# savage-hacker14/audio-to-sheet-music

Hardware: AMD Instinct MI355X
Metric: 6s-segments/sec (each separated into 4 stems; encode once, decode 4x) (higher is better)
Workload: dtype bf16; 1 GPU; BASELINE configs[2]: B=64 x 6 s segments x 4 prompts per GPU; global_batch=64, seq_len=264600, prompts=4, parallelism=segment-sharded dp1, launch=hipGraph replay of one athd_forward_prompts per step (1 graph(s) per rank), pipelines=1, decode_items=256

## Files before the change

### audio-to-sheet-music_amd/csrc/forward.cpp

```cpp
#include "forward.h"

namespace athd_fwd {

int forward_impl(athd_ctx* c, const float* wav, int64_t B, int64_t T, const float* text, bool per_item, int P,
                 float* out, void* ws, size_t ws_bytes, void* stream) {
    if (!c) return ATHD_EINVAL;
    if (!c->finalized) return c->fail(ATHD_ESTATE, "athd_forward before athd_finalize");
    if (!wav || !text || !out || B <= 0 || T <= 0 || P <= 0) return c->fail(ATHD_EINVAL, "bad forward arguments");
    if (P > 256) return c->fail(ATHD_EINVAL, "at most 256 prompts per athd_forward_prompts call");
    if (T > (int64_t)1 << 26) return c->fail(ATHD_EINVAL, "segment too long");
    const Dims d = make_dims(c, B, T, P);
    Bufs b;
    Arena sz;
    const size_t need = plan(sz, d, b, c->mode == 1);
    if (!ws || ws_bytes < need) return c->fail(ATHD_EWORKSPACE, "workspace too small: need " + std::to_string(need));
    Arena ar{(char*)ws};
    plan(ar, d, b, c->mode == 1);
    if (hipSetDevice(c->device) != hipSuccess) return c->fail(ATHD_EHIP, "hipSetDevice failed");
    Run r(c, (hipStream_t)stream, b.stats);
    if (hipMemsetAsync(b.stats, 0, (size_t)b.nstats * 2 * sizeof(double), r.s) != hipSuccess)
        return c->fail(ATHD_EHIP, "memset failed");
    struct ProfBind {
        KProf* saved;
        explicit ProfBind(KProf* p) : saved(t_kprof) { t_kprof = p; }
        ~ProfBind() { t_kprof = saved; }
    } prof_bind(c->prof);
    encode(r, d, b, wav);
    if (r.ok()) transformer(r, d, b);
    for (int64_t ch = 0; ch < d.chunks && r.err == 0; ++ch) {
        const int64_t s0 = ch * d.Bc;
        const int64_t bc = std::min(d.Bc, B - s0);
        decode_chunk(r, d, b, s0, bc, text, per_item, out, (ch & 1) && b.FO2 ? b.FO2 : b.FO);
    }
    if (r.ok()) r.sp.final_join();
    if (d.chunks == 1) dump_all(d, b, r.xt2, r.s);
    if (r.err) return c->fail(ATHD_EHIP, "launch failed in " + r.what + " (code " + std::to_string(r.err) + ")");
    hipError_t e = hipGetLastError();
    if (e != hipSuccess) return c->fail(ATHD_EHIP, std::string("HIP error: ") + hipGetErrorString(e));
    return ATHD_OK;
}

}

using namespace athd_fwd;

extern "C" {

size_t athd_workspace_bytes(athd_ctx* c, int64_t B, int64_t T, int P) {
    if (!c || B <= 0 || T <= 0 || P <= 0) return 0;
    Bufs b;
    Arena a;
    return plan(a, make_dims(c, B, T, P), b, c->mode == 1);
}

int athd_forward(athd_ctx* c, const float* wav, int64_t B, int64_t T, const float* text_emb, float* out, void* ws,
                 size_t ws_bytes, void* stream) {
    return forward_impl(c, wav, B, T, text_emb, true, 1, out, ws, ws_bytes, stream);
}

int athd_forward_prompts(athd_ctx* c, const float* wav, int64_t B, int64_t T, const float* text_table, int P,
                         float* out, void* ws, size_t ws_bytes, void* stream) {
    return forward_impl(c, wav, B, T, text_table, false, P, out, ws, ws_bytes, stream);
}

}
```

### audio-to-sheet-music_amd/csrc/forward.h

```cpp
#pragma once
#include <hip/hip_runtime.h>

#include <algorithm>
#include <cstdio>
#include <cstdlib>
#include <string>
#include <vector>

#include "../../include/athd.h"
#include "attn.h"
#include "ctx.h"
#include "gemm.h"
#include "kernels.h"
#include "prof.h"

namespace athd_fwd {

struct Dims {
    int64_t B = 0, T = 0;
    int P = 1, Tspec = 0;
    int F[5] = {2048, 512, 128, 32, 8};
    int64_t L[5] = {0, 0, 0, 0, 0};
    int64_t Nf = 0, Nt = 0, Nmax = 0;
    int64_t Bc = 0, chunks = 0;
};

struct Bufs {
    float* specT;
    double* stats;
    int64_t nstats;
    float *snorm, *tnorm_div, *tnorm_std;
    void *saved[4], *saved_t[4];
    void *sk4, *sk4t;
    void *ybuf, *ybuf_t;
    float *hbuf, *hbuf_t;
    uint16_t *hbuf_b, *hbuf_b_t;
    int ea = 4;
    float *X, *XT;
    void *H[4], *QKV, *O, *F1;
    void *QKVt, *Ot, *F1t;
    float *Gt, *Dt;
    float *pos2d, *pos1d, *x_enc, *xt_enc;
    uint16_t *x_enc_b, *xt_enc_b;
    float *avec, *tc0, *tc2;
    float *Yb, *x_cond, *xt_cond;
    void* Hm;
    float* Ybt;
    void* Hmt;
    float *G, *D, *FO;
    float* FO2 = nullptr;
    float* ola_part;
    LrStep* lrsteps;
    float* gram;
    double* gramq;
    void *S, *Z, *Zs;
    float* skw[2] = {nullptr, nullptr};
};

inline void* eoff(void* p, int64_t n, int ea) { return (char*)p + n * ea; }

struct Switches {
    static bool env(const char* name, bool dflt) {
        const char* e = std::getenv(name);
        return dflt ? !(e && *e == '0') : (e && *e && *e != '0');
    }
    bool serial = env("ATHD_SERIAL", false), sk = env("ATHD_SK", true), rowln = env("ATHD_ROWLN", true),
         fdec1_fused = env("ATHD_FDEC1_FUSED", true), fenc_row = env("ATHD_FENC_ROW", true);
};

struct Status {
    int err = 0;
    std::string what;
    void check(int rc, const char* w) { if (rc != 0 && err == 0) { err = rc; what = w; } }
};

enum Branch { MAIN = 0, TIME = 1 };
struct StreamPlan {
    hipStream_t main, time;
    hipEvent_t ev_f, ev_t;
    bool serial;
    Status* st;

    StreamPlan(athd_ctx* c, hipStream_t caller, bool serial_, Status* st_)
        : main(caller), time(serial_ ? caller : c->s_time), ev_f(c->ev_f), ev_t(c->ev_t), serial(serial_), st(st_) {
        if (!c->s_time || !c->ev_f || !c->ev_t) st->check((int)hipErrorInvalidResourceHandle, "second stream");
    }
    void record(hipEvent_t ev, hipStream_t s) { st->check((int)hipEventRecord(ev, s), "event record"); }
    void wait(hipStream_t s, hipEvent_t ev) { st->check((int)hipStreamWaitEvent(s, ev, 0), "event wait"); }
    void fork() { record(ev_f, main); wait(time, ev_f); }
    void join() { record(ev_t, time); wait(main, ev_t); }
    void cross_join() {
        record(ev_f, main); record(ev_t, time);
        wait(time, ev_f); wait(main, ev_t);
    }
    void main_into_time() { record(ev_f, main); wait(time, ev_f); }
    void chunk_record_time() { if (!serial) record(ev_t, time); }
    void chunk_wait_time() { if (!serial) wait(main, ev_t); }
    void final_join() { if (!serial) join(); }
};

struct Run : Status {
    athd_ctx* c;
    const Switches sw;
    StreamPlan sp;
    hipStream_t s;
    int sk = 0;
    int mode;
    bool actbf;
    double* st_next;
    float* xt2 = nullptr;

    Run(athd_ctx* c_, hipStream_t caller, double* stats_pool)
        : c(c_), sp(c_, caller, sw.serial || c_->prof != nullptr, this), s(caller), mode(c_->mode),
          actbf(c_->mode == 1), st_next(stats_pool) {}
    bool ok() const { return err == 0; }
    double* stats(int64_t pairs) { double* p = st_next; st_next += 2 * pairs; return p; }
    void gemm(const GemmDesc& g, const char* w) {
        KSite site(w);
        check(gemm_launch(g, mode, s), w);
    }
};

struct OnBranch {
    Run& r;
    const hipStream_t saved_s;
    const int saved_sk;
    OnBranch(Run& r_, Branch b) : r(r_), saved_s(r_.s), saved_sk(r_.sk) {
        r.s = b == TIME ? r.sp.time : r.sp.main;
        r.sk = b == TIME && !r.sp.serial ? 1 : 0;
    }
    ~OnBranch() { r.s = saved_s; r.sk = saved_sk; }
};

inline GemmDesc conv_h(const GemmW& w, const void* A, int a_bf16, int64_t nb, int64_t H_in, int64_t W, int C_in,
                       int ntaps, int in_stride, int in_off, int dil, int64_t H_out) {
    GemmDesc g;
    g.A = A; g.a_bf16 = a_bf16; g.nb = (int)nb; g.H_in = (int)H_in; g.W = (int)W; g.C_in = C_in; g.a_ld = C_in;
    g.ntaps = ntaps; g.in_stride = in_stride; g.in_off = in_off; g.dil = dil; g.H_out = (int)H_out;
    g.Wp = w.w; g.N = w.N; g.K = w.K; g.Kp = w.Kp; g.bias = w.bias;
    return g;
}
inline GemmDesc conv1(const GemmW& w, const void* A, int a_bf16, int64_t nb, int64_t H, int64_t W, int C_in) {
    return conv_h(w, A, a_bf16, nb, H, W, C_in, 1, 1, 0, 1, H);
}
inline void out_to(GemmDesc& g, void* C, int c_bf16, int ldo, int64_t H_out_total) {
    g.C = C; g.c_bf16 = c_bf16; g.ldo = ldo; g.H_out_total = (int)H_out_total;
}
inline GemmDesc lin(const GemmW& w, const void* A, int a_bf16, int64_t nb, int64_t ntok, int ldA, void* C, int c_bf16) {
    GemmDesc g = conv1(w, A, a_bf16, nb, ntok, 1, w.K);
    g.a_ld = ldA;
    out_to(g, C, c_bf16, w.N, ntok);
    return g;
}

Dims make_dims(const athd_ctx* c, int64_t B, int64_t T, int P);
size_t plan(Arena& ar, const Dims& d, Bufs& b, bool actbf);
void dump_all(const Dims& d, const Bufs& b, const float* xt2, hipStream_t s);
void encode(Run& r, const Dims& d, const Bufs& b, const float* wav);
void transformer(Run& r, const Dims& d, const Bufs& b);
void decode_chunk(Run& r, const Dims& d, const Bufs& b, int64_t s0, int64_t Bc, const float* text, bool text_per_item,
                  float* out, float* FO);

}
```

### audio-to-sheet-music_amd/csrc/forward_dec.cpp

```cpp
#include "forward.h"

namespace athd_fwd {
namespace {

void conv_t(Run& r, const DecW& w, const void* A, int a_bf16, int nb, int H_in, int W, void* out, int out_bf16,
            double* st, int keep, const char* stage) {
    KStage kst(stage);
    if (w.ct4w && a_bf16 && out_bf16 && convt4_supported(w.cin, w.cout, nb, H_in, W)) {
        ConvT4Desc q;
        q.x = (const uint16_t*)A; q.w = w.ct4w; q.bias = w.ct4b; q.out = (uint16_t*)out; q.stats = st;
        q.nb = nb; q.H = H_in; q.W = W; q.keep = keep < 0 ? 0 : 1;
        r.check(convt4_launch(q, r.s), "convt4");
        return;
    }
    auto residues = [&](const GemmW& gw, int ntaps, int in_off) {
        GemmDesc g = conv_h(gw, A, a_bf16, nb, H_in, W, w.cin, ntaps, 1, in_off, 1, H_in);
        out_to(g, out, out_bf16, w.cout, (keep < 0 ? 4 : 2) * H_in);
        g.o_stride = keep < 0 ? 4 : 2;
        g.stats = st; g.col_split = w.cout;
        return g;
    };
    if (w.quad.w) {
        GemmDesc g = residues(w.quad, 3, -1);
        if (w.cin % 32 == 0) g.k_blk = w.cin;
        if (keep < 0) { g.o_off = 0; g.store_mask = 15; }
        else { g.o_off = -1; g.store_mask = 6; }
        r.gemm(g, "convt.quad");
        return;
    }
    for (int pi = 0; pi < 2; ++pi) {
        GemmDesc g = residues(w.pair[pi], 2, pi == 0 ? -1 : 0);
        if (keep < 0) { g.o_off = 2 * pi; g.store_mask = 3; }
        else if (pi == 0) { g.o_off = 0; g.hi_row_off = 0; g.store_mask = 2; }
        else { g.o_off = 1; g.store_mask = 1; }
        r.gemm(g, pi == 0 ? "convt.pair01" : "convt.pair23");
    }
}

struct Chunk {
    Run& r;
    const Dims& d;
    const Bufs& b;
    athd_ctx* c;
    int64_t s0, Bc;
    int P, NI, ab;
    void text_attn(const float* enc, const uint16_t* enc_b, int64_t ntok, float* cond, void* Hm, float* Yb) const;
    void last_level(DecLastDesc& dl, const float* fold, const void* skip, int64_t H_skip) const {
        dl.NI = NI; dl.P = P;
        dl.fold = fold; dl.skip = skip; dl.skip_bf16 = ab; dl.H_skip = (int)H_skip; dl.C_skip = 4;
    }
    void freq_decoder(float* FO) const;
    float* time_decoder() const;
};

void Chunk::text_attn(const float* enc, const uint16_t* enc_b, int64_t ntok, float* cond, void* Hm, float* Yb) const {
    KStage kst(ntok == d.Nf ? "text_attn.freq" : "text_attn.time");
    GemmDesc g = lin(c->mlp0, enc_b ? (const void*)enc_b : enc, enc_b ? 1 : 0, Bc, ntok, 384, Hm, ab);
    g.bias = nullptr; g.pbias = b.tc0; g.pfold = P; g.act = ACT_GELU;
    r.gemm(g, "text.mlp0");
    GemmDesc g2 = lin(c->mlp2, Hm, ab, NI, ntok, 384, Yb, 0);
    g2.bias = nullptr; g2.pbias = b.tc2; g2.res = enc; g2.res_div = P; g2.res_bs = ntok * 384;
    if (r.actbf) {
        g2.C = cond; g2.c_bf16 = 1; g2.ln_w = c->ta_nw; g2.ln_b = c->ta_nb;
        r.gemm(g2, "text.mlp2.ln");
        return;
    }
    r.gemm(g2, "text.mlp2");
    LnDesc l;
    l.x = Yb; l.nb = NI; l.N = ntok; l.C = 384; l.w = c->ta_nw; l.b = c->ta_nb; l.out = cond; l.out_bf16 = ab;
    layernorm_launch(l, r.s);
}

void Chunk::freq_decoder(float* FO) const {
    const int64_t Ts = d.Tspec;
    const int ea = b.ea;
    void* const sv[4] = {eoff(b.saved[0], s0 * 512 * Ts * 48, ea), eoff(b.saved[1], s0 * 128 * Ts * 96, ea),
                         eoff(b.saved[2], s0 * 32 * Ts * 192, ea), eoff(b.saved[3], s0 * 8 * Ts * 384, ea)};
    double* st = r.stats(NI);
    conv_t(r, c->fdec[0], b.x_cond, ab, NI, 8, (int)Ts, b.G, ab, st, -1, "fdec0");
    KStage kst("fdec0");
    if (r.actbf)
        gn_gelu_bf16in_launch((const uint16_t*)b.G, (uint16_t*)b.S, NI, 32 * Ts * 192, 192, st, c->fdec[0].gnw,
                              c->fdec[0].gnb, r.s);
    else gn_gelu_launch(b.G, NI, 32 * Ts * 192, 192, st, c->fdec[0].gnw, c->fdec[0].gnb, r.s, false);
    KStage kst1("fdec1");
    const DecW& w1 = c->fdec[1];
    GemmDesc gz = conv1(w1.taps, r.actbf ? b.S : (const void*)b.G, ab, NI, 32, Ts, w1.cin);
    out_to(gz, b.Z, ab, w1.taps.N, 32);
    LowRankDesc lr;
    lr.steps = b.lrsteps;
    lr.Z = b.Z; lr.Zs = b.Zs; lr.z_bf16 = ab; lr.Hs = 32; lr.Hk = 8; lr.Hd = (int)Ts; lr.W = (int)Ts;
    lr.Co = w1.cout; lr.P = P; lr.NI = NI; lr.bias = w1.bias; lr.stats = r.stats(NI);
    lr.gn_w = w1.gnw; lr.gn_b = w1.gnb; lr.fast_gelu = ab;
    lr.skip = sv[2]; lr.skip_bf16 = ab; lr.H_skip = 32; lr.C_skip = 192;
    lr.out = b.D; lr.out_bf16 = ab;
    lr.S = gz.A; lr.Wt = w1.taps.w; lr.w_ld = w1.taps.Kp; lr.Ci = w1.cin;
    const bool gram = r.sw.fdec1_fused && b.gram && fdec1_gram_supported(lr);
    if (gram) { lr.z_taps = 4; lr.z4 = b.Z; }
    else r.gemm(gz, "fdec1.z");
    GemmDesc gs = conv1(w1.taps, sv[3], ab, Bc, 8, Ts, w1.cin);
    gs.a_ld = 384;
    out_to(gs, b.Zs, ab, w1.taps.N, 8);
    r.gemm(gs, "fdec1.zs");
    r.check(fdec_lr_steps_launch(b.lrsteps, (int)Ts, 32, 8, 32, r.s), "fdec_lr_steps");
    if (gram) r.check(fdec1_gram_launch(lr, b.gram, b.gramq, r.s), "fdec1_gram");
    else r.check(fdec_lr_stats_launch(lr, r.s), "fdec_lr_stats");
    r.check(fdec_lr_merge_launch(lr, r.s), "fdec_lr_merge");
    const DecW& w = c->fdec[2];
    double* sti = r.stats(NI);
// ... 85 lines not shown
```

### audio-to-sheet-music_amd/csrc/forward_plan.cpp

```cpp
#include "forward.h"

namespace athd_fwd {

Dims make_dims(const athd_ctx* c, int64_t B, int64_t T, int P) {
    Dims d;
    d.B = B; d.T = T; d.P = P;
    d.Tspec = (int)cdiv(T, 1024);
    d.L[0] = T;
    for (int i = 0; i < 4; ++i) d.L[i + 1] = cdiv(d.L[i], 4);
    d.Nf = 8LL * d.Tspec;
    d.Nt = d.L[4];
    d.Nmax = std::max(d.Nf, d.Nt);
    int64_t items_per_chunk = c ? c->decode_items : 64;
    if (const char* e = std::getenv("ATHD_DECODE_ITEMS")) {
        const long v = std::strtol(e, nullptr, 10);
        if (v > 0) items_per_chunk = v;
    }
    d.Bc = std::max<int64_t>(1, std::min<int64_t>(B, items_per_chunk / P));
    d.chunks = cdiv(B, d.Bc);
    return d;
}

size_t plan(Arena& ar, const Dims& d, Bufs& b, bool actbf) {
    const int64_t B = d.B, Ts = d.Tspec;
// ... 32 lines not shown
    b.hbuf_b = ab == 2 ? ar.take<uint16_t>(hmax) : nullptr;
    b.X = ar.take<float>(B * d.Nf * 512);
    b.XT = ar.take<float>(B * d.Nt * 512);
    for (int i = 0; i < 4; ++i) b.H[i] = act(B * d.Nmax * 512);
    b.QKV = act(B * d.Nmax * 1536);
    b.O = act(B * d.Nmax * 512);
    b.F1 = act(B * d.Nmax * 2048);
    b.QKVt = act(B * d.Nmax * 1536);
    b.Ot = act(B * d.Nt * 512);
    b.F1t = act(B * d.Nt * 2048);
    b.pos2d = ar.take<float>(d.Nf * 512);
    b.pos1d = ar.take<float>(d.Nt * 512);
    b.x_enc = ar.take<float>(B * d.Nf * 384);
    b.xt_enc = ar.take<float>(B * d.Nt * 384);
    b.x_enc_b = actbf ? ar.take<uint16_t>(B * d.Nf * 384) : nullptr;
    b.xt_enc_b = actbf ? ar.take<uint16_t>(B * d.Nt * 384) : nullptr;
    const int64_t NI = d.Bc * d.P;
    b.avec = ar.take<float>(NI * 384);
    b.tc0 = ar.take<float>(NI * 384);
    b.tc2 = ar.take<float>(NI * 384);
    b.Hm = act(NI * d.Nf * 384);
    b.Yb = ar.take<float>(NI * d.Nf * 384);
    b.Hmt = act(NI * d.Nt * 384);
    b.Ybt = ar.take<float>(NI * d.Nt * 384);
    b.x_cond = ar.take<float>(NI * d.Nf * 384);
    b.xt_cond = ar.take<float>(NI * d.Nt * 384);
    const int64_t gt = std::max<int64_t>({4 * d.Nt * 192, 4 * d.L[3] * 96, 4 * d.L[2] * 48, d.T * 2});
    const int64_t dmt = std::max<int64_t>({d.L[3] * 192, d.L[2] * 96, d.L[1] * 48});
    b.G = ar.take<float>(NI * std::max<int64_t>({32 * Ts * 192, 2 * Ts * Ts * 96, gt}));
    b.D = ar.take<float>(NI * std::max<int64_t>(Ts * Ts * 192, dmt));
    b.Gt = ar.take<float>(NI * gt);
    b.Dt = ar.take<float>(NI * dmt);
    b.S = act(NI * 32 * Ts * DEC_CH[1]);
    b.Z = act(NI * 32 * Ts * 8 * DEC_CH[2]);
    b.Zs = act(d.Bc * 8 * Ts * 8 * DEC_CH[2]);
    b.FO = ar.take<float>(NI * Ts * Ts * 2);
    if (d.chunks > 1) b.FO2 = ar.take<float>(NI * Ts * Ts * 2);
    b.ola_part = ar.take<float>(istft_ola_part_floats(NI, (int)Ts));
    b.lrsteps = ar.take<LrStep>(Ts + 1);
    b.gram = actbf ? ar.take<float>(fdec1_gram_floats(NI, (int)Ts)) : nullptr;
    b.gramq = actbf ? ar.take<double>(fdec1_gram_q_doubles()) : nullptr;
    for (int i = 0; i < 2; ++i) b.skw[i] = actbf ? ar.take<float>(SK_WS_BYTES / 4) : nullptr;
    return ar.off;
}

static bool dump_dev(const char* dir, const std::string& name, const void* p, size_t n) {
    std::vector<char> h(n);
    if (hipMemcpy(h.data(), p, n, hipMemcpyDeviceToHost) != hipSuccess) return false;
    FILE* f = std::fopen((std::string(dir) + "/" + name).c_str(), "wb");
    if (f) { std::fwrite(h.data(), 1, n, f); std::fclose(f); }
    return true;
}

void dump_all(const Dims& d, const Bufs& b, const float* xt2, hipStream_t s) {
    const char* dir = std::getenv("ATHD_DUMP");
    if (!dir || !*dir) return;
    if (hipStreamSynchronize(s) != hipSuccess) return;
    const int64_t B = d.B, Ts = d.Tspec, NI = std::min(d.B, d.Bc) * d.P;
    struct E { std::string name; const void* p; int64_t n; std::string shape; };
    std::vector<E> es = {
        {"specT", b.specT, B * Ts * 2048 * 4, "B,Ts,2048,4"},
        {"snorm", b.snorm, 2 * B, "B,2"}, {"tnorm_std", b.tnorm_std, 2 * B, "B,2"},
        {"x_enc", b.x_enc, B * d.Nf * 384, "B,Nf,384"}, {"xt_enc", b.xt_enc, B * d.Nt * 384, "B,Nt,384"},
        {"x_cond", b.x_cond, NI * d.Nf * 384, "NI,Nf,384"}, {"xt_cond", b.xt_cond, NI * d.Nt * 384, "NI,Nt,384"},
        {"FO", b.FO, NI * Ts * Ts * 2, "NI,t,row,2"}, {"XT2", xt2, NI * d.T * 2, "NI,T,2"},
    };
    for (int i = 0; i < 4; ++i) {
        const std::string si = std::to_string(i);
        const int64_t nf = B * d.F[i + 1] * Ts * ENC_CH[i], nt = B * d.L[i + 1] * ENC_CH[i];
        if (b.ea == 4) {
            es.push_back({"saved" + si, b.saved[i], nf, "B,F,Ts,C"});
            es.push_back({"saved_t" + si, b.saved_t[i], nt, "B,L,C"});
        } else {
            dump_dev(dir, "saved" + si + ".bf16", b.saved[i], (size_t)nf * 2);
            dump_dev(dir, "saved_t" + si + ".bf16", b.saved_t[i], (size_t)nt * 2);
        }
    }
    struct Rw { const char* name; const void* p; const void* end; };
    const Rw rws[] = {{"G", b.G, b.D}, {"D", b.D, b.Gt}, {"Gt", b.Gt, b.Dt}, {"Dt", b.Dt, b.S}, {"S", b.S, b.Z},
                      {"Z", b.Z, b.Zs}, {"Zs", b.Zs, b.FO}, {"stats", b.stats, b.specT}};
    for (const auto& e : rws)
        if (e.p && e.end && e.end > e.p)
            dump_dev(dir, std::string(e.name) + ".raw", e.p, (size_t)((const char*)e.end - (const char*)e.p));
    FILE* fi = std::fopen((std::string(dir) + "/index.txt").c_str(), "w");
    for (const auto& e : es)
        if (dump_dev(dir, e.name + ".f32", e.p, (size_t)e.n * 4) && fi)
            std::fprintf(fi, "%s %lld %s\n", e.name.c_str(), (long long)e.n, e.shape.c_str());
    if (fi) std::fclose(fi);
}

}
```

### audio-to-sheet-music_amd/csrc/forward_xf.cpp

```cpp
#include "forward.h"

namespace athd_fwd {
namespace {

struct Pending { const double* st = nullptr; const float* w = nullptr; const float* b = nullptr; };

struct BranchX {
    float* X;
    int64_t N;
    void *QKV, *O, *F1;
    Pending pend;
    Pending resgn;
};

struct Xf {
    Run& r;
    const Dims& d;
    const Bufs& b;
    const int ab;

    void ln(BranchX& x, const float* w, const float* bb, bool pending, void* out, const float* w2 = nullptr,
            const float* b2 = nullptr, void* out2 = nullptr) {
        LnDesc l;
        l.x = x.X; l.nb = (int)d.B; l.N = x.N; l.C = 512; l.w = w; l.b = bb; l.out = out; l.out_bf16 = ab;
// ... 6 lines not shown
        l.w2 = w2; l.b2 = b2; l.out2 = out2;
        layernorm_launch(l, r.s);
    }
    void block(const TLayerW& L, BranchX& x, void* Hq, void* Hkv, int64_t Nk) {
        const int64_t B = d.B, N = x.N;
        AttnDesc a;
        a.nb = (int)B; a.Nq = (int)N; a.Nk = (int)Nk; a.heads = 8;
        a.scale = r.actbf ? ATTN_SCALE_PRESCALED : 0.125f;
        if (!L.cross) {
            r.gemm(lin(L.qkv, Hq, ab, B, N, 512, x.QKV, ab), "qkv");
            a.Q = x.QKV; a.q_bf16 = ab; a.q_bs = N * 1536; a.q_ld = 1536; a.q_off = 0;
            a.K = x.QKV; a.k_bf16 = ab; a.k_bs = N * 1536; a.k_ld = 1536; a.k_off = 512;
            a.V = x.QKV; a.v_bf16 = ab; a.v_bs = N * 1536; a.v_ld = 1536; a.v_off = 1024;
        } else {
            char* Qb = (char*)x.QKV;
            char* KVb = Qb + (size_t)B * d.Nmax * 512 * (ab ? 2 : 4);
            r.gemm(lin(L.q, Hq, ab, B, N, 512, Qb, ab), "q");
            r.gemm(lin(L.kv, Hkv, ab, B, Nk, 512, KVb, ab), "kv");
            a.Q = Qb; a.q_bf16 = ab; a.q_bs = N * 512; a.q_ld = 512; a.q_off = 0;
            a.K = KVb; a.k_bf16 = ab; a.k_bs = Nk * 1024; a.k_ld = 1024; a.k_off = 0;
            a.V = KVb; a.v_bf16 = ab; a.v_bs = Nk * 1024; a.v_ld = 1024; a.v_off = 512;
        }
        a.O = x.O; a.o_bf16 = ab; a.o_bs = N * 512; a.o_ld = 512;
        r.check(attn_launch(a, r.mode, r.s), "attention");
        GemmDesc go = lin(L.out, x.O, ab, B, N, 512, x.X, 0);
        go.res = x.X; go.res_scale = L.g1;
        if (x.resgn.st) {
            go.res_gn_stats = x.resgn.st; go.res_gn_count = N * 512; go.res_gn_w = x.resgn.w; go.res_gn_b = x.resgn.b;
            x.resgn = Pending();
        }
        const float *n2w = L.cross ? L.n3w : L.n2w, *n2b = L.cross ? L.n3b : L.n2b;
        go.ln_w = n2w; go.ln_b = n2b; go.ln_out = Hq;
        if (r.actbf && r.sw.rowln && rowln_supported(go)) {
            r.gemm(go, "out_proj.ln");
        } else {
            go.ln_w = go.ln_b = nullptr; go.ln_out = nullptr;
            r.gemm(go, "out_proj");
            ln(x, n2w, n2b, false, Hq);
        }
        GemmDesc g1 = lin(L.l1, Hq, ab, B, N, 512, x.F1, ab);
        g1.act = ACT_GELU;
        r.gemm(g1, "linear1");
        double* st = r.stats(B);
        GemmDesc g2 = lin(L.l2, x.F1, ab, B, N, 2048, x.X, 0);
        g2.res = x.X; g2.res_scale = L.g2; g2.stats = st;
        g2.sk_ws = r.sw.sk ? b.skw[r.sk] : nullptr;
        r.gemm(g2, "linear2");
        x.pend.st = st; x.pend.w = L.now; x.pend.b = L.nob;
    }
    void down(const GemmW& w, BranchX& x, float* enc, uint16_t* enc_b, const char* site) {
        GemmDesc g = lin(w, x.X, 0, d.B, x.N, 512, enc, 0);
        if (r.actbf) { g.a_gn_stats = x.pend.st; g.a_gn_count = x.N * 512; g.a_gn_w = x.pend.w; g.a_gn_b = x.pend.b; }
        r.gemm(g, site);
        if (enc_b) to_bf16_launch(enc, enc_b, d.B * x.N * 384, r.s);
    }
};

}

void transformer(Run& r, const Dims& d, const Bufs& b) {
    athd_ctx* c = r.c;
    KStage xstage("transformer");
    KSection sec_x("transformer");
    const int64_t B = d.B;
    Xf xf{r, d, b, r.actbf ? 1 : 0};
    BranchX f{b.X, d.Nf, b.QKV, b.O, b.F1}, t{b.XT, d.Nt, b.QKVt, b.Ot, b.F1t};
    r.gemm(lin(c->up, b.saved[3], xf.ab, B, d.Nf, 384, b.X, 0), "upsampler");
    r.gemm(lin(c->up_t, b.saved_t[3], xf.ab, B, d.Nt, 384, b.XT, 0), "upsampler_t");
    pos2d_launch(b.pos2d, 8, d.Tspec, 512, r.s);
    pos1d_launch(b.pos1d, (int)d.Nt, 512, r.s);
    LnDesc l;
    l.x = b.X; l.nb = (int)B; l.N = d.Nf; l.C = 512; l.w = c->nin_w; l.b = c->nin_b; l.pos = b.pos2d; l.out = b.X;
    layernorm_launch(l, r.s);
    LnDesc lt;
    lt.x = b.XT; lt.nb = (int)B; lt.N = d.Nt; lt.C = 512; lt.w = c->nint_w; lt.b = c->nint_b; lt.pos = b.pos1d; lt.out = b.XT;
    layernorm_launch(lt, r.s);
    if (!r.ok()) return;
    r.sp.fork();
    for (int idx = 0; idx < 5; ++idx) {
        const TLayerW& Lf = c->L[idx];
        const TLayerW& Lt = c->Lt[idx];
        if (!Lf.cross) {
            xf.ln(f, Lf.n1w, Lf.n1b, true, b.H[0]);
            xf.block(Lf, f, b.H[0], nullptr, d.Nf);
            OnBranch on(r, TIME);
            xf.ln(t, Lt.n1w, Lt.n1b, true, b.H[2]);
            xf.block(Lt, t, b.H[2], nullptr, d.Nt);
        } else {
            r.sp.cross_join();
            xf.ln(f, Lf.n1w, Lf.n1b, true, b.H[0], Lt.n2w, Lt.n2b, b.H[1]);
            {
                OnBranch on(r, TIME);
                xf.ln(t, Lt.n1w, Lt.n1b, true, b.H[2], Lf.n2w, Lf.n2b, b.H[3]);
            }
            r.sp.cross_join();
            xf.block(Lf, f, b.H[0], b.H[3], d.Nt);
            OnBranch on(r, TIME);
            xf.block(Lt, t, b.H[2], b.H[1], d.Nf);
        }
    }
    if (!r.actbf) gn_apply_launch(b.X, (int)B, d.Nf, 512, f.pend.st, f.pend.w, f.pend.b, r.s);
    {
        OnBranch on(r, TIME);
        if (!r.actbf) gn_apply_launch(b.XT, (int)B, d.Nt, 512, t.pend.st, t.pend.w, t.pend.b, r.s);
        xf.down(c->down_t, t, b.xt_enc, b.xt_enc_b, "downsampler_t");
    }
    xf.down(c->down, f, b.x_enc, b.x_enc_b, "downsampler");
// ... 5 lines not shown
```

### audio-to-sheet-music_amd/csrc/kernels.h

```cpp
#pragma once
#include <hip/hip_runtime.h>
#include <stdint.h>

#include "gemm.h"

namespace athd {

struct PadPlan {
    int64_t L;
    int64_t left;
    int64_t ext_left;
    int64_t Lx;
};
inline PadPlan stft_pad_plan(int64_t T, int64_t Tspec) {
    const int64_t pl = 1536, pr = 1536 + Tspec * 1024 - T, maxpad = pl > pr ? pl : pr;
    const int64_t extra = T <= maxpad ? maxpad - T + 1 : 0, epr = pr < extra ? pr : extra, epl = extra - epr;
    PadPlan pp;
    pp.L = T; pp.left = pl - epl; pp.ext_left = epl; pp.Lx = T + epl + epr;
    return pp;
}

void tconv0_launch(const float* wav, int nb, int64_t T, int64_t Lo, const float* w, const float* bias,
                   const float* tnorm, void* out, int out_bf16, hipStream_t s);

void stft_launch(const float* wav, int nb, int64_t T, const PadPlan& pp, int Tspec, const float2* tw,
                 const double2* tw64, const float* win, float* specT, double* stats, hipStream_t s);
void istft_ola_launch(const float* fo, int NI, int Tspec, int P, int64_t T, const float* spec, const float2* tw,
                      const double2* tw64, const float* win, const float* win2, const float* xt2, const float* tnorm,
                      float* out, float* part, hipStream_t s);
int istft_ola_nwg(int Tspec);
int istft_ola_frames(int Tspec);
inline int64_t istft_ola_part_floats(int64_t NI, int Tspec) { return NI * istft_ola_nwg(Tspec) * 2 * 3 * 1024 * 2; }

void stats_launch(const float* x, int nb, int64_t n, double* stats, hipStream_t s);
void input_norm_params_launch(const double* stats, int nb, int64_t n, float* mean_inv, float* mean_std,
                              hipStream_t s);
void gn_gelu_launch(float* h, int nb, int64_t per_batch, int H, const double* stats, const float* w,
                    const float* b, hipStream_t s, bool fast);
void gn_gelu_bf16_launch(const float* h, uint16_t* out, int nb, int64_t per_batch, int H, const double* stats,
                         const float* w, const float* b, hipStream_t s);
void gn_gelu_bf16in_launch(const uint16_t* h, uint16_t* out, int nb, int64_t per_batch, int H, const double* stats,
                           const float* w, const float* b, hipStream_t s);
void gn_apply_launch(float* x, int nb, int64_t N, int C, const double* stats, const float* w, const float* b,
                     hipStream_t s);
struct LnDesc {
    float* x = nullptr; int nb = 1; int64_t N = 0; int C = 512;
    const float* w = nullptr; const float* b = nullptr;
    const double* gn_stats = nullptr; const float* gn_w = nullptr; const float* gn_b = nullptr;
    int gn_writeback = 1;
    const float* pos = nullptr;
    void* out = nullptr; int out_bf16 = 0;
    const float* w2 = nullptr; const float* b2 = nullptr; void* out2 = nullptr;
};
inline bool ln_lazy_gn_ok(const LnDesc& d) { return d.C == 512 && (!d.out2 || (d.out_bf16 && !d.pos)); }

void layernorm_launch(const LnDesc& d, hipStream_t s);
void to_bf16_launch(const float* x, uint16_t* y, int64_t n, hipStream_t s);
void text_vec_launch(const float* text, int NI, int P, int text_per_item, const float* maT, const float* ma,
                     const float* mcT, const float* mc, const float* b2, float* a, float* c0, float* c2, hipStream_t s);
struct MergeDesc {
    const void* src = nullptr; int src_bf16 = 0; int H_src = 0;
    int kept = 0;
    int C = 0;
    const double* stats = nullptr; int64_t gn_count = 0; const float* gn_w = nullptr; const float* gn_b = nullptr;
    const void* skip = nullptr; int skip_bf16 = 0; int H_skip = 0; int C_skip = 0; int P = 1;
    void* out = nullptr; int out_bf16 = 0; int H_out = 0; int W = 1; int NI = 1;
    const float* proj_w = nullptr; const float* proj_b = nullptr;
    int fast_gelu = 0;
};
int dec_merge_launch(const MergeDesc& d, hipStream_t s);
void pos2d_launch(float* out, int Fr, int T1, int C, hipStream_t s);
void pos1d_launch(float* out, int T2, int C, hipStream_t s);
struct LrStep {
    float lz, lk, lj;
    uint32_t zk;
    uint32_t jj;
    uint32_t flags;
    uint32_t pad[2];
};
struct LowRankDesc {
    const LrStep* steps = nullptr;
    const void* Z = nullptr; const void* Zs = nullptr; int z_bf16 = 0;
    int z_taps = 8;
    int Hs = 32, Hk = 8, Hd = 0, W = 0, Co = 0, P = 1, NI = 0;
    const float* bias = nullptr;
    double* stats = nullptr;
    const float* gn_w = nullptr; const float* gn_b = nullptr; int fast_gelu = 0;
    const void* skip = nullptr; int skip_bf16 = 0; int H_skip = 0; int C_skip = 0;
    void* out = nullptr; int out_bf16 = 0;
    const void* S = nullptr;
    const void* Wt = nullptr; int w_ld = 0;
    int Ci = 0;
    void* z4 = nullptr;
};
int fdec_lr_steps_launch(LrStep* steps, int Hd, int Hs, int Hk, int H_skip, hipStream_t s);
int fdec_lr_stats_launch(const LowRankDesc& d, hipStream_t s);
int fdec_lr_merge_launch(const LowRankDesc& d, hipStream_t s);
bool fdec1_gram_supported(const LowRankDesc& d);
int64_t fdec1_gram_floats(int64_t NI, int W);
int64_t fdec1_gram_q_doubles();
int fdec1_gram_launch(const LowRankDesc& d, float* gram, double* gq, hipStream_t s);
constexpr int FR_MT_MAX = 17;
struct FencRowDesc {
    const void* in = nullptr;
    const float* a_norm = nullptr;
    int B = 0, Fin = 0, Fout = 0, T = 0;
    const uint16_t* wc = nullptr; int wc_ld = 0; const float* bc = nullptr;
    const uint16_t* w3[2] = {nullptr, nullptr}; int w3_ld = 0;
    const float* b3[2] = {nullptr, nullptr};
    const float* g1w[2] = {nullptr, nullptr}; const float* g1b[2] = {nullptr, nullptr};
    const uint16_t* w1[2] = {nullptr, nullptr}; int w1_ld = 0;
    const float* b1[2] = {nullptr, nullptr};
// ... 109 lines not shown
```

### audio-to-sheet-music_amd/csrc/ktest.cpp

```cpp
#include <hip/hip_runtime.h>
#include <stdint.h>
#include <string.h>

#include "attn.h"
#include "ctx.h"
#include "gemm.h"
#include "kernels.h"
#include "text_tower.h"

namespace athd {
int dec_merge_run();
int dec_merge_maxp();
int dec_last_const(int which);
int fdec1_gram_wb();
int fdec1_gram_blocks();
}

using namespace athd;

extern "C" {

struct KtGemm {
    void* A; int64_t a_bf16, nb, H_in, W, C_in, a_ld, a_cs, a_bs, a_hs, ntaps, in_stride, in_off, dil, H_out;
    void* a_norm; void* a_gn_stats; int64_t a_gn_count; void* a_gn_w; void* a_gn_b;
    void* Wp; int64_t N, K, Kp; void* bias;
    void* C; int64_t c_bf16, H_out_total, o_stride, o_off, ldo, col_off, c_bs, store; void* c4;
    int64_t col_split, hi_row_off, store_mask, k_blk, act;
    void* res; int64_t res_bf16; void* res_scale; void* res_gn_stats; int64_t res_gn_count; void* res_gn_w; void* res_gn_b;
    void* row_add; void* stats; void* gn_stats; int64_t gn_count; void* gn_w; void* gn_b;
    void* pbias; int64_t pfold, res_div, res_bs;
    void* ln_w; void* ln_b; void* ln_out; void* sk_ws;
};

struct KtAttn {
    void* Q; int64_t q_bf16, q_bs, q_ld, q_off;
    void* K; int64_t k_bf16, k_bs, k_ld, k_off;
    void* V; int64_t v_bf16, v_bs, v_ld, v_off;
    void* O; int64_t o_bf16, o_bs, o_ld;
    int64_t nb, Nq, Nk, heads;
    int64_t scale_bits;
};

struct KtLn {
    void* x; int64_t nb, N, C; void* w; void* b; void* gn_stats; void* gn_w; void* gn_b; int64_t gn_writeback;
    void* pos; void* out; int64_t out_bf16; void* w2; void* b2; void* out2;
};

struct KtConvT4 {
    void* x; void* w; void* bias; void* out; void* stats; int64_t nb, H, W, keep;
};

struct KtConv3 {
    void* x; void* w; int64_t kp; void* bias; void* h; void* st; int64_t M, L, C, dil;
};

struct KtApply {
    void* hb; void* w; int64_t kp; void* bias; void* st; void* gn_w; void* gn_b; void* scale; void* x; int64_t M, L, C;
    int64_t rewrite; void* rw_w; int64_t rw_kp; void* rw_bias; void* rw_out; void* rw_c4;
// ... 307 lines not shown
    if (rc != 0) return rc;
    return tt_attn_launch((const float*)d->part, (int)d->S, (const float*)d->bias, (const int32_t*)d->mask, (int)d->P,
                          (int)d->L, (float*)d->out, (hipStream_t)stream);
}

struct KtStft {
    void* wav; int64_t nb, T, Tspec; void* tw; void* tw64; void* win; void* specT; void* stats;
    int64_t pp_L, pp_left, pp_ext_left, pp_Lx;
};
struct KtIstft {
    void* fo; int64_t NI, Tspec, P, T; void* spec; void* tw; void* tw64; void* win; void* win2; void* xt2; void* tnorm;
    void* out; void* part;
};
struct KtTconv0 { void* wav; int64_t nb, T, Lo; void* w; void* bias; void* tnorm; void* out; int64_t out_bf16; };
struct KtTextVec {
    void* text; int64_t NI, P, per_item; void* maT; void* ma; void* mcT; void* mc; void* b2; void* a; void* c0; void* c2;
};
int64_t kt_sizeof_stft() { return (int64_t)sizeof(KtStft); }
int64_t kt_sizeof_istft() { return (int64_t)sizeof(KtIstft); }
int64_t kt_sizeof_tconv0() { return (int64_t)sizeof(KtTconv0); }
int64_t kt_sizeof_textvec() { return (int64_t)sizeof(KtTextVec); }

int kt_stft(const KtStft* k, void* stream) {
    PadPlan pp;
    pp.L = k->pp_L; pp.left = k->pp_left; pp.ext_left = k->pp_ext_left; pp.Lx = k->pp_Lx;
    stft_launch((const float*)k->wav, (int)k->nb, k->T, pp, (int)k->Tspec, (const float2*)k->tw, (const double2*)k->tw64,
                (const float*)k->win, (float*)k->specT, (double*)k->stats, (hipStream_t)stream);
    return (int)hipGetLastError();
}
void kt_stft_pad_plan(int64_t T, int64_t Tspec, int64_t* out4) {
    const PadPlan pp = stft_pad_plan(T, Tspec);
    out4[0] = pp.L; out4[1] = pp.left; out4[2] = pp.ext_left; out4[3] = pp.Lx;
}
int kt_istft_ola(const KtIstft* k, void* stream) {
    istft_ola_launch((const float*)k->fo, (int)k->NI, (int)k->Tspec, (int)k->P, k->T, (const float*)k->spec,
                     (const float2*)k->tw, (const double2*)k->tw64, (const float*)k->win, (const float*)k->win2,
                     (const float*)k->xt2, (const float*)k->tnorm, (float*)k->out, (float*)k->part, (hipStream_t)stream);
    return (int)hipGetLastError();
}
int64_t kt_istft_nwg(int64_t Tspec) { return istft_ola_nwg((int)Tspec); }
int64_t kt_istft_frames(int64_t Tspec) { return istft_ola_frames((int)Tspec); }
int64_t kt_istft_part_floats(int64_t NI, int64_t Tspec) { return istft_ola_part_floats(NI, (int)Tspec); }
int kt_tconv0(const KtTconv0* k, void* stream) {
    tconv0_launch((const float*)k->wav, (int)k->nb, k->T, k->Lo, (const float*)k->w, (const float*)k->bias,
                  (const float*)k->tnorm, k->out, (int)k->out_bf16, (hipStream_t)stream);
    return (int)hipGetLastError();
}
int kt_text_vec(const KtTextVec* k, void* stream) {
    text_vec_launch((const float*)k->text, (int)k->NI, (int)k->P, (int)k->per_item, (const float*)k->maT,
                    (const float*)k->ma, (const float*)k->mcT, (const float*)k->mc, (const float*)k->b2, (float*)k->a,
                    (float*)k->c0, (float*)k->c2, (hipStream_t)stream);
    return (int)hipGetLastError();
}
int kt_pos2d(float* out, int64_t Fr, int64_t T1, int64_t C, void* stream) {
    pos2d_launch(out, (int)Fr, (int)T1, (int)C, (hipStream_t)stream);
    return (int)hipGetLastError();
}
int kt_pos1d(float* out, int64_t T2, int64_t C, void* stream) {
    pos1d_launch(out, (int)T2, (int)C, (hipStream_t)stream);
    return (int)hipGetLastError();
}

}
```

Before: 1887 segments/s.

## Fuse text-conditioning MLP, residual and LayerNorm into one per-tile kernel

Adds a single HIP kernel that, for each tile of encoder tokens, converts the fp32 activations to bf16 in LDS and runs the first MLP GEMM once. It then applies the per-prompt bias and GELU, runs the second GEMM, and does the residual add and LayerNorm for every prompt, writing the conditioned bf16 output directly. This replaces the separate mlp0/mlp2 GEMM launches, the LayerNorm pass, the intermediate Hm buffer round trips and the standalone bf16 conversion of the encoder output, so the first GEMM is shared across all prompts. In exchange the kernel uses a large fixed LDS footprint and heavy register tiling, which can limit occupancy. It applies only to bf16 mode with C=384.

```diff
diff --git a/audio-to-sheet-music_amd/csrc/forward.cpp b/audio-to-sheet-music_amd/csrc/forward.cpp
--- a/audio-to-sheet-music_amd/csrc/forward.cpp
+++ b/audio-to-sheet-music_amd/csrc/forward.cpp
@@ -18,6 +18,7 @@
     plan(ar, d, b, c->mode == 1);
     if (hipSetDevice(c->device) != hipSuccess) return c->fail(ATHD_EHIP, "hipSetDevice failed");
     Run r(c, (hipStream_t)stream, b.stats);
+    r.text_fused = text_stage_decide(c, r.sw, d, b, r.actbf);
     if (hipMemsetAsync(b.stats, 0, (size_t)b.nstats * 2 * sizeof(double), r.s) != hipSuccess)
         return c->fail(ATHD_EHIP, "memset failed");
     struct ProfBind {
@@ -31,6 +32,7 @@
         const int64_t s0 = ch * d.Bc;
         const int64_t bc = std::min(d.Bc, B - s0);
         decode_chunk(r, d, b, s0, bc, text, per_item, out, (ch & 1) && b.FO2 ? b.FO2 : b.FO);
+        if (d.chunks > 1 && r.ok()) dump_chunk_cond(d, b, ch, bc);
     }
     if (r.ok()) r.sp.final_join();
     if (d.chunks == 1) dump_all(d, b, r.xt2, r.s);
diff --git a/audio-to-sheet-music_amd/csrc/forward.h b/audio-to-sheet-music_amd/csrc/forward.h
--- a/audio-to-sheet-music_amd/csrc/forward.h
+++ b/audio-to-sheet-music_amd/csrc/forward.h
@@ -65,7 +65,8 @@
         return dflt ? !(e && *e == '0') : (e && *e && *e != '0');
     }
     bool serial = env("ATHD_SERIAL", false), sk = env("ATHD_SK", true), rowln = env("ATHD_ROWLN", true),
-         fdec1_fused = env("ATHD_FDEC1_FUSED", true), fenc_row = env("ATHD_FENC_ROW", true);
+         fdec1_fused = env("ATHD_FDEC1_FUSED", true), fenc_row = env("ATHD_FENC_ROW", true),
+         text_fused = env("ATHD_TEXT_FUSED", true) && std::getenv("ATHD_RLT") == nullptr;
 };
 
 struct Status {
@@ -107,6 +108,7 @@
     int sk = 0;
     int mode;
     bool actbf;
+    bool text_fused = false;
     double* st_next;
     float* xt2 = nullptr;
 
@@ -153,9 +155,26 @@
     return g;
 }
 
+inline athd::TextStageDesc text_stage_desc(const athd_ctx* c, const Bufs& b, bool actbf, const float* enc, int64_t Bc,
+                                           int64_t ntok, int P, void* cond) {
+    athd::TextStageDesc t;
+    t.x = enc; t.W0 = (const uint16_t*)c->mlp0.w; t.W2 = (const uint16_t*)c->mlp2.w;
+    t.N = c->mlp0.N == c->mlp2.N ? c->mlp0.N : 0; t.K = c->mlp0.K == c->mlp2.K ? c->mlp0.K : 0;
+    t.Kp = c->mlp0.Kp; t.Kp2 = c->mlp2.Kp;
+    t.c0 = b.tc0; t.c2 = b.tc2; t.ln_w = c->ta_nw; t.ln_b = c->ta_nb; t.out = (uint16_t*)cond;
+    t.Bc = (int)Bc; t.P = P; t.ntok = ntok; t.bf16_mode = actbf ? 1 : 0;
+    return t;
+}
+inline bool text_stage_decide(const athd_ctx* c, const Switches& sw, const Dims& d, const Bufs& b, bool actbf) {
+    return actbf && sw.text_fused &&
+           athd::text_stage_supported(text_stage_desc(c, b, actbf, b.x_enc, d.Bc, d.Nf, d.P, b.x_cond)) &&
+           athd::text_stage_supported(text_stage_desc(c, b, actbf, b.xt_enc, d.Bc, d.Nt, d.P, b.xt_cond));
+}
+
 Dims make_dims(const athd_ctx* c, int64_t B, int64_t T, int P);
 size_t plan(Arena& ar, const Dims& d, Bufs& b, bool actbf);
 void dump_all(const Dims& d, const Bufs& b, const float* xt2, hipStream_t s);
+void dump_chunk_cond(const Dims& d, const Bufs& b, int64_t ch, int64_t bc);
 void encode(Run& r, const Dims& d, const Bufs& b, const float* wav);
 void transformer(Run& r, const Dims& d, const Bufs& b);
 void decode_chunk(Run& r, const Dims& d, const Bufs& b, int64_t s0, int64_t Bc, const float* text, bool text_per_item,
diff --git a/audio-to-sheet-music_amd/csrc/forward_dec.cpp b/audio-to-sheet-music_amd/csrc/forward_dec.cpp
--- a/audio-to-sheet-music_amd/csrc/forward_dec.cpp
+++ b/audio-to-sheet-music_amd/csrc/forward_dec.cpp
@@ -55,6 +55,11 @@
 
 void Chunk::text_attn(const float* enc, const uint16_t* enc_b, int64_t ntok, float* cond, void* Hm, float* Yb) const {
     KStage kst(ntok == d.Nf ? "text_attn.freq" : "text_attn.time");
+    if (r.text_fused) {
+        KSite site("text.fused");
+        r.check(text_stage_launch(text_stage_desc(c, b, r.actbf, enc, Bc, ntok, P, cond), r.s), "text.fused");
+        return;
+    }
     GemmDesc g = lin(c->mlp0, enc_b ? (const void*)enc_b : enc, enc_b ? 1 : 0, Bc, ntok, 384, Hm, ab);
     g.bias = nullptr; g.pbias = b.tc0; g.pfold = P; g.act = ACT_GELU;
     r.gemm(g, "text.mlp0");
diff --git a/audio-to-sheet-music_amd/csrc/forward_plan.cpp b/audio-to-sheet-music_amd/csrc/forward_plan.cpp
--- a/audio-to-sheet-music_amd/csrc/forward_plan.cpp
+++ b/audio-to-sheet-music_amd/csrc/forward_plan.cpp
@@ -108,6 +108,15 @@
     return true;
 }
 
+void dump_chunk_cond(const Dims& d, const Bufs& b, int64_t ch, int64_t bc) {
+    const char* dir = std::getenv("ATHD_DUMP");
+    if (!dir || !*dir) return;
+    if (hipDeviceSynchronize() != hipSuccess) return;
+    const std::string tag = ".c" + std::to_string(ch) + ".raw";
+    dump_dev(dir, "x_cond" + tag, b.x_cond, (size_t)(bc * d.P * d.Nf * 384) * b.ea);
+    dump_dev(dir, "xt_cond" + tag, b.xt_cond, (size_t)(bc * d.P * d.Nt * 384) * b.ea);
+}
+
 void dump_all(const Dims& d, const Bufs& b, const float* xt2, hipStream_t s) {
     const char* dir = std::getenv("ATHD_DUMP");
     if (!dir || !*dir) return;
diff --git a/audio-to-sheet-music_amd/csrc/forward_xf.cpp b/audio-to-sheet-music_amd/csrc/forward_xf.cpp
--- a/audio-to-sheet-music_amd/csrc/forward_xf.cpp
+++ b/audio-to-sheet-music_amd/csrc/forward_xf.cpp
@@ -82,7 +82,7 @@
         GemmDesc g = lin(w, x.X, 0, d.B, x.N, 512, enc, 0);
         if (r.actbf) { g.a_gn_stats = x.pend.st; g.a_gn_count = x.N * 512; g.a_gn_w = x.pend.w; g.a_gn_b = x.pend.b; }
         r.gemm(g, site);
-        if (enc_b) to_bf16_launch(enc, enc_b, d.B * x.N * 384, r.s);
+        if (enc_b && !r.text_fused) to_bf16_launch(enc, enc_b, d.B * x.N * 384, r.s);
     }
 };
 
diff --git a/audio-to-sheet-music_amd/csrc/kernels.h b/audio-to-sheet-music_amd/csrc/kernels.h
--- a/audio-to-sheet-music_amd/csrc/kernels.h
+++ b/audio-to-sheet-music_amd/csrc/kernels.h
@@ -58,6 +58,20 @@
 void to_bf16_launch(const float* x, uint16_t* y, int64_t n, hipStream_t s);
 void text_vec_launch(const float* text, int NI, int P, int text_per_item, const float* maT, const float* ma,
                      const float* mcT, const float* mc, const float* b2, float* a, float* c0, float* c2, hipStream_t s);
+struct TextStageDesc {
+    const float* x = nullptr;
+    const uint16_t* W0 = nullptr; const uint16_t* W2 = nullptr;
+    int N = 0, K = 0, Kp = 0, Kp2 = 0;
+    const float* c0 = nullptr; const float* c2 = nullptr;
+    const float* ln_w = nullptr; const float* ln_b = nullptr;
+    uint16_t* out = nullptr;
+    int Bc = 0, P = 0;
+    int64_t ntok = 0;
+    int bf16_mode = 0;
+};
+int text_stage_bm();
+bool text_stage_supported(const TextStageDesc& d);
+int text_stage_launch(const TextStageDesc& d, hipStream_t s);
 struct MergeDesc {
     const void* src = nullptr; int src_bf16 = 0; int H_src = 0;
     int kept = 0;
diff --git a/audio-to-sheet-music_amd/csrc/ktest.cpp b/audio-to-sheet-music_amd/csrc/ktest.cpp
--- a/audio-to-sheet-music_amd/csrc/ktest.cpp
+++ b/audio-to-sheet-music_amd/csrc/ktest.cpp
@@ -4,6 +4,7 @@
 
 #include "attn.h"
 #include "ctx.h"
+#include "forward.h"
 #include "gemm.h"
 #include "kernels.h"
 #include "text_tower.h"
@@ -417,6 +418,23 @@
                     (float*)k->c0, (float*)k->c2, (hipStream_t)stream);
     return (int)hipGetLastError();
 }
+struct KtTextStage {
+    void* x; void* W0; void* W2; int64_t N, K, Kp, Kp2; void* c0; void* c2; void* ln_w; void* ln_b; void* out;
+    int64_t Bc, P, ntok, bf16_mode;
+};
+static TextStageDesc text_stage_desc(const KtTextStage* k) {
+    TextStageDesc d;
+    d.x = (const float*)k->x; d.W0 = (const uint16_t*)k->W0; d.W2 = (const uint16_t*)k->W2;
+    d.N = (int)k->N; d.K = (int)k->K; d.Kp = (int)k->Kp; d.Kp2 = (int)k->Kp2;
+    d.c0 = (const float*)k->c0; d.c2 = (const float*)k->c2; d.ln_w = (const float*)k->ln_w; d.ln_b = (const float*)k->ln_b;
+    d.out = (uint16_t*)k->out; d.Bc = (int)k->Bc; d.P = (int)k->P; d.ntok = k->ntok; d.bf16_mode = (int)k->bf16_mode;
+    return d;
+}
+int64_t kt_sizeof_textstage() { return (int64_t)sizeof(KtTextStage); }
+int64_t kt_text_stage_bm() { return text_stage_bm(); }
+int kt_text_stage_supported(const KtTextStage* k) { return text_stage_supported(text_stage_desc(k)) ? 1 : 0; }
+int kt_text_stage(const KtTextStage* k, void* stream) { return text_stage_launch(text_stage_desc(k), (hipStream_t)stream); }
+int kt_text_fused_switch() { return athd_fwd::Switches().text_fused ? 1 : 0; }
 int kt_pos2d(float* out, int64_t Fr, int64_t T1, int64_t C, void* stream) {
     pos2d_launch(out, (int)Fr, (int)T1, (int)C, (hipStream_t)stream);
     return (int)hipGetLastError();
diff --git a/audio-to-sheet-music_amd/csrc/text_stage.hip b/audio-to-sheet-music_amd/csrc/text_stage.hip
--- /dev/null
+++ b/audio-to-sheet-music_amd/csrc/text_stage.hip
@@ -0,0 +1,251 @@
+#include "gemm_tile.h"
+#include "kernels.h"
+#include "prof.h"
+
+namespace athd {
+
+namespace {
+
+constexpr int TS_C = 384;
+constexpr int TS_NW = 8, TS_TN = TS_C / TS_NW / 16;
+constexpr int TS_KS = TS_C / 32, TS_KT = TS_C / 64;
+#ifndef ATHD_TS_BM
+#define ATHD_TS_BM 112
+#endif
+constexpr int TS_BM = ATHD_TS_BM;
+
+}
+
+template <int BM>
+__global__ __launch_bounds__(64 * TS_NW, 2) void text_stage_kernel(const TextStageDesc d) {
+    constexpr int NT = 64 * TS_NW, NW = TS_NW, TN = TS_TN, C = TS_C;
+    constexpr int TM = BM / 16, STAGE = BM * LDS_ROWB;
+    static_assert(BM % 16 == 0 && TN * 16 * NW == C, "tile shape");
+    __shared__ __attribute__((aligned(1024))) char img[TS_KT * STAGE];
+    __shared__ __attribute__((aligned(16))) float pc[2][4][C];
+    __shared__ __attribute__((aligned(16))) float pln[2][C];
+    __shared__ __attribute__((aligned(16))) float red[2][BM][NW];
+
+    const int tid = threadIdx.x, lane = tid & 63;
+    const int wave = __builtin_amdgcn_readfirstlane(tid >> 6);
+    const int l15 = lane & 15, l4 = lane >> 4;
+    const uint32_t rps = (uint32_t)d.ntok;
+    const uint32_t M = (uint32_t)d.Bc * rps;
+    const int P = d.P;
+    const int ntm = (int)((M + BM - 1) / BM);
+    const int tile = xcd_remap((int)blockIdx.x, (int)gridDim.x);
+    if (tile >= ntm) return;
+    const uint32_t m0 = (uint32_t)tile * BM;
+    const int n0 = TN * 16 * wave;
+    const uint32_t b0 = m0 / rps;
+    const uint32_t b1 = (b0 + 1) * rps < M ? b0 + 1 : b0;
+    const uint32_t m1 = (b0 + 1) * rps;
+
+    auto load_pc = [&](int p) {
+        for (int i = tid; i < 4 * C; i += NT) {
+            const int k = i / C, n = i % C;
+            const float* src = (k < 2 ? d.c0 : d.c2) + ((int64_t)((k & 1) ? b1 : b0) * P + p) * C;
+            pc[p & 1][k][n] = src[n];
+        }
+    };
+    for (int i = tid; i < 2 * C; i += NT) pln[i / C][i % C] = (i < C ? d.ln_w : d.ln_b)[i % C];
+    load_pc(0);
+
+    {
+        constexpr int NCH = BM * (C / 8), NQ = (NCH + NT - 1) / NT;
+        float4 xa[NQ], xb[NQ];
+#pragma unroll
+        for (int q = 0; q < NQ; ++q) {
+            const int ch = tid + NT * q, row = ch / (C / 8), cc = ch % (C / 8);
+            const uint32_t m = m0 + row;
+            xa[q] = xb[q] = make_float4(0.f, 0.f, 0.f, 0.f);
+            if (ch < NCH && m < M) {
+                const float4* src = reinterpret_cast<const float4*>(d.x + (int64_t)m * C + 8 * cc);
+                xa[q] = src[0];
+                xb[q] = src[1];
+            }
+        }
+#pragma unroll
+        for (int q = 0; q < NQ; ++q) {
+            const int ch = tid + NT * q, row = ch / (C / 8), cc = ch % (C / 8);
+            if (ch < NCH)
+                *reinterpret_cast<uint4*>(img + (cc >> 3) * STAGE + row * LDS_ROWB + (((cc & 7) ^ (row & 7)) * 16)) =
+                    make_uint4(pack2bf(xa[q].x, xa[q].y), pack2bf(xa[q].z, xa[q].w), pack2bf(xb[q].x, xb[q].y),
+                               pack2bf(xb[q].z, xb[q].w));
+        }
+    }
+
+    const int woff = (n0 + l15) * d.Kp + 8 * l4;
+    const char* arow = img + l15 * LDS_ROWB;
+    auto kloop = [&](const bf16_t* W, f32x4_t (&acc)[TM][TN]) {
+        bf16x8_t bq[2][TN];
+#pragma unroll
+        for (int j = 0; j < TN; ++j) bq[0][j] = *reinterpret_cast<const bf16x8_t*>(W + woff + 16 * j * d.Kp);
+#pragma unroll
+        for (int ks = 0; ks < TS_KS; ++ks) {
+            const int kt = ks / 2, s = ks % 2;
+            if (ks + 1 < TS_KS) {
+#pragma unroll
+                for (int j = 0; j < TN; ++j)
+                    bq[(ks + 1) & 1][j] = *reinterpret_cast<const bf16x8_t*>(W + woff + 16 * j * d.Kp + 32 * (ks + 1));
+            }
+            bf16x8_t af[TM];
+#pragma unroll
+            for (int i = 0; i < TM; ++i)
+                af[i] = *reinterpret_cast<const bf16x8_t*>(arow + kt * STAGE + i * 16 * LDS_ROWB + swz_slot(s, l4, l15));
+#pragma unroll
+            for (int i = 0; i < TM; ++i)
+#pragma unroll
+                for (int j = 0; j < TN; ++j)
+                    acc[i][j] = __builtin_amdgcn_mfma_f32_16x16x32_bf16(bq[ks & 1][j], af[i], acc[i][j], 0, 0, 0);
+            __builtin_amdgcn_sched_barrier(0);
+        }
+    };
+
+    f32x4_t acc1[TM][TN];
+#pragma unroll
+    for (int i = 0; i < TM; ++i)
+#pragma unroll
+        for (int j = 0; j < TN; ++j) acc1[i][j] = f32x4_t{0.f, 0.f, 0.f, 0.f};
+    __syncthreads();
+    kloop(d.W0, acc1);
+
+    const int cl = n0 + 4 * l4;
+    const auto row_total = [&](int buf, int row) {
+        float t = 0.f;
+#pragma unroll
+        for (int w = 0; w < NW; w += 4) {
+            const float4 a = *reinterpret_cast<const float4*>(&red[buf][row][w]);
+            t += (a.x + a.y) + (a.z + a.w);
+        }
+        return t;
+    };
+
+    for (int p = 0; p < P; ++p) {
+        const int par = p & 1;
+        __syncthreads();
+        if (p + 1 < P) load_pc(p + 1);
+        int rl = l15, cw = cl;
+        asm volatile("" : "+v"(rl), "+v"(cw));
+#pragma unroll
+        for (int i = 0; i < TM; ++i) {
+            const int row = 16 * i + rl;
+            const bool second = m0 + row >= m1;
+#pragma unroll
+            for (int j = 0; j < TN; ++j) {
+                const int c = cw + 16 * j;
+                const float4 c0 = *reinterpret_cast<const float4*>(&pc[par][second ? 1 : 0][c]);
+                const athd_f2v g01 = gelu_fast_pk((athd_f2v){acc1[i][j][0] + c0.x, acc1[i][j][1] + c0.y});
+                const athd_f2v g23 = gelu_fast_pk((athd_f2v){acc1[i][j][2] + c0.z, acc1[i][j][3] + c0.w});
+                *reinterpret_cast<uint2*>(img + (c >> 6) * STAGE + row * LDS_ROWB + ((((c & 63) >> 3) ^ (row & 7)) * 16) +
+                                          (c & 7) * 2) = make_uint2(pack2bf(g01.x, g01.y), pack2bf(g23.x, g23.y));
+            }
+        }
+        f32x4_t acc[TM][TN];
+#pragma unroll
+        for (int i = 0; i < TM; ++i)
+#pragma unroll
+            for (int j = 0; j < TN; ++j) acc[i][j] = f32x4_t{0.f, 0.f, 0.f, 0.f};
+        __syncthreads();
+        kloop(d.W2, acc);
+
+        float rs[TM];
+        asm volatile("" : "+v"(rl), "+v"(cw));
+#pragma unroll
+        for (int i = 0; i < TM; ++i) {
+            const uint32_t m = m0 + 16 * i + rl;
+            const uint32_t mm = m < M ? m : M - 1;
+            const bool second = m >= m1;
+            const float* R = d.x + (int64_t)mm * C + cw;
+            float4 r[TN];
+#pragma unroll
+            for (int j = 0; j < TN; ++j) r[j] = *reinterpret_cast<const float4*>(R + 16 * j);
+            float sum = 0.f;
+#pragma unroll
+            for (int j = 0; j < TN; ++j) {
+                const float4 pb = *reinterpret_cast<const float4*>(&pc[par][second ? 3 : 2][cw + 16 * j]);
+                acc[i][j][0] = r[j].x + (acc[i][j][0] + pb.x);
+                acc[i][j][1] = r[j].y + (acc[i][j][1] + pb.y);
+                acc[i][j][2] = r[j].z + (acc[i][j][2] + pb.z);
+                acc[i][j][3] = r[j].w + (acc[i][j][3] + pb.w);
+                sum += (acc[i][j][0] + acc[i][j][1]) + (acc[i][j][2] + acc[i][j][3]);
+            }
+            rs[i] = sum;
+        }
+#pragma unroll
+        for (int i = 0; i < TM; ++i) {
+            rs[i] += __shfl_xor(rs[i], 16, 64);
+            rs[i] += __shfl_xor(rs[i], 32, 64);
+        }
+        if (l4 == 0) {
+#pragma unroll
+            for (int i = 0; i < TM; ++i) red[0][16 * i + l15][wave] = rs[i];
+        }
+        __syncthreads();
+        float mean[TM];
+#pragma unroll
+        for (int i = 0; i < TM; ++i) {
+            mean[i] = row_total(0, 16 * i + l15) * (1.f / C);
+            float q = 0.f;
+#pragma unroll
+            for (int j = 0; j < TN; ++j)
+#pragma unroll
+                for (int e = 0; e < 4; ++e) {
+                    const float dv = acc[i][j][e] - mean[i];
+                    q += dv * dv;
+                }
+            q += __shfl_xor(q, 16, 64);
+            q += __shfl_xor(q, 32, 64);
+            rs[i] = q;
+        }
+        if (l4 == 0) {
+#pragma unroll
+            for (int i = 0; i < TM; ++i) red[1][16 * i + l15][wave] = rs[i];
+        }
+        __syncthreads();
+        asm volatile("" : "+v"(rl), "+v"(cw));
+#pragma unroll
+        for (int i = 0; i < TM; ++i) {
+            const float rstd = 1.f / sqrtf(row_total(1, 16 * i + rl) * (1.f / C) + 1e-5f);
+            const uint32_t m = m0 + 16 * i + rl;
+            if (m >= M) continue;
+            const uint32_t seg = m >= m1 ? b1 : b0;
+            bf16_t* out = d.out + (((int64_t)seg * P + p) * rps + (m - seg * rps)) * C;
+#pragma unroll
+            for (int j = 0; j < TN; ++j) {
+                const int c = cw + 16 * j;
+                const float4 lw = *reinterpret_cast<const float4*>(&pln[0][c]);
+                const float4 lb = *reinterpret_cast<const float4*>(&pln[1][c]);
+                const float y0 = (acc[i][j][0] - mean[i]) * rstd * lw.x + lb.x;
+                const float y1 = (acc[i][j][1] - mean[i]) * rstd * lw.y + lb.y;
+                const float y2 = (acc[i][j][2] - mean[i]) * rstd * lw.z + lb.z;
+                const float y3 = (acc[i][j][3] - mean[i]) * rstd * lw.w + lb.w;
+                *reinterpret_cast<uint2*>(out + c) = make_uint2(pack2bf(y0, y1), pack2bf(y2, y3));
+            }
+        }
+    }
+}
+
+int text_stage_bm() { return TS_BM; }
+
+bool text_stage_supported(const TextStageDesc& d) {
+    const auto al16 = [](const void* p) { return p && ((uintptr_t)p & 15) == 0; };
+    return d.bf16_mode && d.N == TS_C && d.K == TS_C && d.Kp >= TS_C && d.Kp % 8 == 0 && d.Kp <= 4096 && d.Kp2 == d.Kp && d.P >= 1 &&
+           d.Bc >= 1 && d.ntok >= TS_BM && (int64_t)d.Bc * d.ntok < (int64_t)1 << 31 && al16(d.x) && al16(d.W0) &&
+           al16(d.W2) && al16(d.c0) && al16(d.c2) && al16(d.ln_w) && al16(d.ln_b) && al16(d.out);
+}
+
+int text_stage_launch(const TextStageDesc& d, hipStream_t s) {
+    if (!text_stage_supported(d)) return -2;
+    const int64_t M = (int64_t)d.Bc * d.ntok;
+    const int ntm = (int)((M + TS_BM - 1) / TS_BM);
+    KScope ks(s);
+    if (ks.on()) {
+        ks.begin("text_stage_kernel", 2.0 * M * TS_C * TS_C * (1 + d.P),
+                 (double)M * TS_C * 4 + (double)M * d.P * TS_C * 2 + 2.0 * TS_C * TS_C * 2);
+    }
+    hipLaunchKernelGGL((text_stage_kernel<TS_BM>), dim3((unsigned)ntm), dim3(64 * TS_NW), 0, s, d);
+    return (int)hipGetLastError();
+}
+
+}
```

Result: no change. 1882 segments/s (-0.3%).
